# theori-io/nrsc5

Measured on AMD Instinct MI355X. Metric: IQ MS/s demod+decoded, higher is better.
Workload: dtype exact float32 half-band (== int16 Q15) / f32 OFDM + sync / int32 Viterbi metrics

## Files before the change

### nrsc5_amd/csrc/engine.hip

```cpp
#include <math.h>
#include <stdarg.h>
#include <stdio.h>
#include <stdlib.h>
#include <algorithm>
#include <atomic>
#include <new>
#include "engine_internal.h"

static_assert(sizeof(nrsc5hip_record) == sizeof(BlockRecord), "record ABI mismatch");
static_assert(sizeof(BlockRecord) % 8 == 0, "record alignment");

static thread_local char g_err[512] = "";
extern "C" const char *nrsc5hip_last_error(void) { return g_err; }
void nrsc5::set_last_error(const char *msg) { snprintf(g_err, sizeof(g_err), "%s", msg); }
int nrsc5::fail(int code, const char *fmt, ...)
{
    char m[sizeof(g_err)];
    va_list ap; va_start(ap, fmt); vsnprintf(m, sizeof(m), fmt, ap); va_end(ap);
    set_last_error(m);
    return code;
}
#ifndef NRSC5HIP_SOURCE_SHA
#define NRSC5HIP_SOURCE_SHA "unknown"
#endif
// ... 293 lines not shown
            if ((rc = dev_alloc(e, &db.l2_ring, S * (size_t)cfg->p1_slots))) break;
            if (hipMemset(db.l2_ring, 0, S * (size_t)cfg->p1_slots * sizeof(nrsc5hip_l2_frame)) != hipSuccess) { rc = NRSC5HIP_EHIP; break; }
            const size_t npx = S * (size_t)db.px_slots * 2, nam = cfg->am_enable ? S * (size_t)cfg->p1_slots * 9 : 0;
            if ((rc = dev_alloc(e, &db.l2_px_ring, npx))) break;
            if (hipMemset(db.l2_px_ring, 0, npx * sizeof(nrsc5hip_l2_frame)) != hipSuccess) { rc = NRSC5HIP_EHIP; break; }
            if (nam) {
                if ((rc = dev_alloc(e, &db.l2_am_ring, nam))) break;
                if (hipMemset(db.l2_am_ring, 0, nam * sizeof(nrsc5hip_l2_frame)) != hipSuccess) { rc = NRSC5HIP_EHIP; break; }
            }
        }
        db.am = nullptr; db.am_sym = nullptr; db.am_q = nullptr; db.am_vit = nullptr; db.am_dec = nullptr; db.am_k9meta = nullptr; db.am_job = nullptr; db.am_ckpt = nullptr; db.am_ber = nullptr; db.am_pids_stage = nullptr; db.am_pids_rec = nullptr; db.am_nvit = 1;
        if (cfg->am_enable) {
            if ((rc = dev_alloc(e, &db.am, S))) break;
            if ((rc = dev_alloc(e, &db.am_sym, S * 4 * AM_SYMS))) break;
            if ((rc = dev_alloc(e, &db.am_q, S * 3 * 2 * (size_t)AM_VIT))) break;
            db.am_nvit = cfg->p1_async ? NWIN : 1;
            const size_t ndec = cfg->p1_async ? NAUX : 1;
            if ((rc = dev_alloc(e, &db.am_vit, S * db.am_nvit * 2 * AM_VIT))) break;
            if ((rc = dev_alloc(e, &db.am_dec, ndec * S * (size_t)(8 * AM_DEC_P1 + AM_DEC_P3)))) break;
            if (cfg->p1_async && (rc = dev_alloc(e, &db.am_k9meta, ndec * S))) break;
            if ((rc = dev_alloc(e, &db.am_job, S * NWIN))) break;
            if ((rc = dev_alloc(e, &db.am_ber, S * (size_t)cfg->p1_slots))) break;
            if (cfg->p1_async && cfg->l2_feedback && (rc = dev_alloc(e, &db.am_ckpt, S * NWIN * 8))) break;
            if ((rc = dev_alloc(e, &db.am_pids_stage, S * NWIN * 8 * (size_t)(3 * PIDS_LEN)))) break;
            if ((rc = dev_alloc(e, &db.am_pids_rec, S * NWIN * 8))) break;
            if (hipMemset(db.am_pids_rec, 0xff, S * NWIN * 8 * sizeof(int)) != hipSuccess) { rc = NRSC5HIP_EHIP; break; }
            if (hipMemset(db.am_job, 0, S * NWIN * sizeof(AmJob)) != hipSuccess || hipMemset(db.am_ber, 0, S * (size_t)cfg->p1_slots * sizeof(float)) != hipSuccess) { rc = NRSC5HIP_EHIP; break; }
            std::vector<AmStream> ainit(S);
            for (size_t k = 0; k < S; k++) init_am_state(ainit[k]);
            if (hipMemcpy(db.am, ainit.data(), S * sizeof(AmStream), hipMemcpyHostToDevice) != hipSuccess ||
                hipMemset(db.am_q, 0, S * 3 * 2 * (size_t)AM_VIT) != hipSuccess || hipMemset(db.am_vit, 0, S * db.am_nvit * 2 * AM_VIT) != hipSuccess ||
                hipMemset(db.am_sym, 0, S * 4 * AM_SYMS) != hipSuccess) { rc = NRSC5HIP_EHIP; snprintf(g_err, sizeof(g_err), "AM state init failed"); break; }
        }
        db.sync_phase_cycles = nullptr;
        e->stage_bytes = 4u << 20; e->stage_ring_bytes = 1u << 20;
        if ((rc = dev_alloc(e, &e->stage_dev, e->stage_bytes))) break;
        if (!cfg->p1_async) {
            for (int k = 0; k < nrsc5hip_engine::NSTAGE && !rc; k++) {
                if ((rc = dev_alloc(e, &e->stage_dev2[k], e->stage_ring_bytes + 16))) break;
                void *sp = nullptr;
                if (hipHostMalloc((void **)&e->stage_pin[k], e->stage_ring_bytes + 16, hipHostMallocMapped) != hipSuccess ||
                    hipHostGetDevicePointer(&sp, e->stage_pin[k], 0) != hipSuccess ||
                    hipEventCreateWithFlags(&e->stage_ev[k], hipEventDisableTiming) != hipSuccess) { rc = NRSC5HIP_ENOMEM; snprintf(g_err, sizeof(g_err), "pinned staging allocation failed"); }
                e->stage_pin_dev[k] = (uint8_t *)sp;
                e->stage_busy[k] = false;
            }
            if (rc) break;
            if (S * (size_t)cfg->p1_slots <= 64) {
                const size_t nw = S * (size_t)cfg->p1_slots * P1_WORDS;
                void *mp = nullptr;
                if (hipHostMalloc((void **)&e->frames_host, nw * sizeof(uint32_t), hipHostMallocMapped) != hipSuccess ||
                    hipHostGetDevicePointer(&mp, e->frames_host, 0) != hipSuccess) { rc = NRSC5HIP_ENOMEM; snprintf(g_err, sizeof(g_err), "pinned frame mirror allocation failed"); break; }
                memset(e->frames_host, 0, nw * sizeof(uint32_t));
                db.p1_mirror = (uint32_t *)mp;
            }
            int prio_least = 0, prio_greatest = 0;
            (void)hipDeviceGetStreamPriorityRange(&prio_least, &prio_greatest);
            if (hipStreamCreateWithPriority(&e->ingest, hipStreamDefault, prio_greatest) != hipSuccess || hipEventCreateWithFlags(&e->ev_ingest, hipEventDisableTiming) != hipSuccess ||
                hipEventCreateWithFlags(&e->ev_main, hipEventDisableTiming) != hipSuccess ||
                hipEventCreateWithFlags(&e->ev_appended, hipEventDisableTiming) != hipSuccess) { rc = NRSC5HIP_EHIP; snprintf(g_err, sizeof(g_err), "ingest stream creation failed"); break; }
            e->ingest_dirty = false; e->main_stepped = false; e->main_appended = false; e->early_flush = 128u << 10;
            if ((rc = dev_alloc(e, &e->decim_ticket, 1))) break;
            if (hipMemset(e->decim_ticket, 0, sizeof(unsigned)) != hipSuccess) { rc = NRSC5HIP_EHIP; break; }
            for (int k = 0; k < 2 && !rc; k++) {
                void *dp = nullptr;
                if (hipHostMalloc((void **)&e->report_host[k], sizeof(StreamReport), hipHostMallocMapped) != hipSuccess ||
                    hipHostGetDevicePointer(&dp, e->report_host[k], 0) != hipSuccess) { rc = NRSC5HIP_ENOMEM; snprintf(g_err, sizeof(g_err), "pinned report allocation failed"); break; }
// ... 230 lines not shown
```

### nrsc5_amd/csrc/engine_stage.hip

```cpp
#include <algorithm>
#include <cmath>
#include "engine_internal.h"

extern "C" void nrsc5hip_debug_seam_totals(double out[8], int reset)
{
    for (int k = 0; k < 8; k++) { if (out) out[k] = g_seam[k]; if (reset) g_seam[k] = 0; }
}
extern "C" void nrsc5hip_debug_seam_counts(double out[6], int reset)
{
    for (int k = 0; k < 6; k++) { if (out) out[k] = g_seam[8 + k]; if (reset) g_seam[8 + k] = 0; }
}

extern "C" int nrsc5hip_stage_l2_index(nrsc5hip_engine *e, const uint8_t *bits, int nbits, int nframes, nrsc5hip_l2_frame *out, uint8_t *pdu_bytes, long long stride)
{
    ON_ENGINE_DEVICE(e);
    if (!e || !bits || !out || nbits < 1 || nframes < 1) FAIL(NRSC5HIP_EINVAL, "bad argument");
    const int words = (nbits + 31) / 32;
    std::vector<uint32_t> w((size_t)words * nframes, 0u);
    for (int f = 0; f < nframes; f++)
        for (int i = 0; i < nbits; i++) w[(size_t)f * words + (i >> 5)] |= (uint32_t)(bits[(size_t)f * nbits + i] & 1u) << (i & 31);
    DevTmp tw;
    HIPCHK(hipMalloc(&tw.p, w.size() * sizeof(uint32_t)));
    uint32_t *dw = (uint32_t *)tw.p;
    HIPCHK(hipMemcpy(dw, w.data(), w.size() * sizeof(uint32_t), hipMemcpyHostToDevice));
// ... 663 lines not shown
    case NRSC5HIP_TUNE_DEFER_WAIT:        e->defer_wait = value != 0; break;
    case NRSC5HIP_TUNE_DIRECT_DECIMATE:   e->direct_decimate = value != 0; break;
    case NRSC5HIP_TUNE_HOST_CAPTURE: {
        if (e->hc_stream >= 0) { int rc = hc_detach(e); if (rc) return rc; }
        if (!e->hc_pin) break;
        e->host_capture = value != 0;
        if (value >= 512) {
            uint8_t *np = nullptr; void *dp = nullptr;
            if (hipHostMalloc((void **)&np, (size_t)value << 10, hipHostMallocMapped) != hipSuccess || hipHostGetDevicePointer(&dp, np, 0) != hipSuccess) FAIL(NRSC5HIP_ENOMEM, "pinned capture allocation failed");
            (void)hipHostFree(e->hc_pin);
            e->hc_pin = np; e->hc_dev = (uint8_t *)dp; e->hc_cap = (size_t)value << 10;
        }
        break;
    }
    case NRSC5HIP_TUNE_MIXFFT_SYMS: {
        e->mixfft_syms = (value == 2 || value == 4 || value == 8 || value == 16 || value == 32 || (value >= 100 && value <= 140)) ? value : 1;
        if (e->mixfft_syms >= 100) {
            int lds_max = 65536;
#ifndef HIPEMU
            HIPCHK(hipDeviceGetAttribute(&lds_max, hipDeviceAttributeMaxSharedMemoryPerBlock, e->cfg.device));
#endif
            const int room_kib = (lds_max - 24 * 1024) / 1024;
            if (e->mixfft_syms - 100 > room_kib) e->mixfft_syms = 100 + std::max(room_kib, 0);
        }
        break;
    }
    case NRSC5HIP_TUNE_AM_SEGMENTS:       e->am_segments = std::min(std::max(value, 1), K9_GMAX); break;
    case NRSC5HIP_TUNE_AM_WARM:           e->am_warm = value > 0 ? K9_WARM : 0; e->am_runin = value > 0 ? K9_TB_RUNIN : 0; break;
    case NRSC5HIP_TUNE_SYNC_PHASES:
        if (value && !e->sync_phase_buf) {
            int rc = dev_alloc(e, &e->sync_phase_buf, 16); if (rc) return rc;
            HIPCHK(hipMemset(e->sync_phase_buf, 0, 16 * sizeof(long long)));
        }
        e->db.sync_phase_cycles = value ? e->sync_phase_buf : nullptr;
        break;
    default: FAIL(NRSC5HIP_EINVAL, "unknown knob %d", knob);
    }
    return 0;
}

extern "C" int nrsc5hip_debug_flow_stats(nrsc5hip_engine *e, long long stats[2])
{
    if (!e || !stats) return NRSC5HIP_EINVAL;
    stats[0] = e->flow_bursts; stats[1] = e->flow_steps;
    return 0;
}

extern "C" int nrsc5hip_debug_host_capture_stats(nrsc5hip_engine *e, long long stats[5])
{
    if (!e || !stats) return NRSC5HIP_EINVAL;
    stats[0] = e->hc_attaches; stats[1] = e->hc_detaches; stats[2] = e->hc_rebases; stats[3] = e->hc_stream; stats[4] = e->reports_folded;
    return 0;
}

extern "C" int nrsc5hip_debug_fwd_stats(nrsc5hip_engine *e, int stats[2])
{
    ON_ENGINE_DEVICE(e);
    if (!e || !stats) FAIL(NRSC5HIP_EINVAL, "null argument");
    HIPCHK(hipDeviceSynchronize());
    HIPCHK(hipMemcpy(stats, e->db.fwd_stats, 2 * sizeof(int), hipMemcpyDeviceToHost));
    return 0;
}

extern "C" int nrsc5hip_debug_tb_stats(nrsc5hip_engine *e, int stats[2])
{
    ON_ENGINE_DEVICE(e);
    if (!stats) FAIL(NRSC5HIP_EINVAL, "null argument");
// ... 24 lines not shown
```

### nrsc5_amd/csrc/kernels.h

```cpp
#pragma once
#include "nrsc5hip.h"
#include "nrsc5_dev.h"

namespace nrsc5 {

struct DevTables {
    const uint16_t *deint_lut;
    const uint16_t *pids_gather;
    const uint32_t *eq_cell;
    const uint16_t *eq_out;
    const uint32_t *scr_p1;
    const uint32_t *scr_pids;
    const float2 *twiddle;
    const float2 *twiddle_a;
    const float *shape;
    const int16_t *hb_q15;
    const int16_t *acq_q15;
    const uint32_t *px_delay_wide;
    const uint32_t *px_delay_narrow;
    const uint32_t *am_deint_p1;
    const uint32_t *am_deint_p3_ma3;
    const uint32_t *am_deint_p3_ma1;
    const int16_t *am_acq_q15;
    const float *am_shape;
// ... 1 lines not shown
};

struct DevBuffers {
    StreamState *state;
    StreamState *ckpt;
    c16 *q15;
    long long q15_cap;
    c16 *acq_win;
    c16 *acq_filt;
    int *acq_list;
    float2 *acq_sums;
    float2 *bins;
    float2 *cfo_snap;
    float *cfo_phase;
    int loop_exact;
    float2 *nco_tab;
    int nco_policy;
    int8_t *pm;
    int8_t *pids_stage;
    int *pids_rec;
    int *coded;
    uint32_t *dec;
    int nstreams_alloc;
    uint8_t *tbmap;
    int *fwd_meta;
    int *fwd_stats;
    int *tb_stats;
    uint32_t *p1_ring;
    uint32_t *p1_mirror;
    int p1_slots;
    BlockRecord *records;
    int rec_cap;
    int *counters;
    long long *sync_phase_cycles;
    int8_t *px_mem;
    int8_t *px_pair;
    int8_t *px_stage;
    PxJob *px_job;
    unsigned long long *px_dec;
    uint32_t *px_ring;
    int px_slots;
    AmStream *am;
    uint8_t *am_sym;
    uint8_t *am_q;
    int8_t *am_vit;
    int am_nvit;
    unsigned long long *am_dec;
    K9Meta *am_k9meta;
    unsigned *am_k9stats;
    AmJob *am_job;
    AmCkpt *am_ckpt;
    float *am_ber;
    int8_t *am_pids_stage;
    int *am_pids_rec;
    nrsc5hip_l2_frame *l2_ring;
    nrsc5hip_l2_frame *l2_px_ring;
    nrsc5hip_l2_frame *l2_am_ring;
};

struct StreamReport { int counters[4]; long long rd; int nblocks; int nrec; BlockRecord rec[4]; unsigned seq; unsigned pad; };
void launch_decimate_fm_cu8_stream(const DevTables &tb, const DevBuffers &db, int s, const uint8_t *iq, unsigned nbytes, unsigned *ticket, hipStream_t st);
void launch_stream_tail(const DevTables &tb, const DevBuffers &db, int s, int first_rec, StreamReport *out, unsigned seq, int do_pids, hipStream_t st);

void launch_decimate_fm_cu8(const DevTables &tb, const DevBuffers &db, int nstreams, const int *stream_ids,
                            const uint8_t *iq_base, long long iq_stride, const unsigned *nbytes, unsigned max_nbytes,
                            hipStream_t st);
// ... 107 lines not shown
```

### nrsc5_amd/csrc/sync_body.h

```cpp
#pragma once
#include <hip/hip_runtime.h>
#include "kernels.h"
#include "wave_ops.h"
#include "viterbi_wave.h"
#include "prepare_block.h"
#include "l2_header.h"
#include "fastmath.h"

namespace nrsc5 {

constexpr int NREF_MAX = 30;
constexpr int CFO_LO = -2 * PW, CFO_HI = 2 * PW;

__device__ inline int ref_bin(int r) { const int i = r >> 1; return (r & 1) ? UB1 - PW * i : LB0 + PW * i; }

constexpr uint32_t PAT_POS = (1u << 1) | (1u << 5) | (1u << 6) | (1u << 8) | (1u << 21);
constexpr uint32_t PAT_NEG = (1u << 0) | (1u << 2) | (1u << 3) | (1u << 4) | (1u << 9) | (1u << 13) | (1u << 14) | (1u << 20) | (1u << 22) | (1u << 31);
constexpr uint32_t NEEDLE_MASK = 0x7fu | (0xfu << 8) | (3u << 13) | (7u << 20) | (1u << 31);
constexpr uint32_t NEEDLE_VAL0 = (1u << 1) | (1u << 5) | (1u << 6) | (1u << 8) | (1u << 21);
__device__ inline uint32_t needle_val(unsigned rsid) { return NEEDLE_VAL0 | ((rsid >> 1) << 10) | ((((rsid >> 1) ^ rsid) & 1u) << 11); }

struct LoopGains { float alpha, beta; };
__device__ inline LoopGains loop_gains()
{
// ... 178 lines not shown

__device__ __forceinline__ float cell_error(float2 v)
{
    const float ix = v.x >= 0 ? 1.0f : -1.0f, iy = v.y >= 0 ? 1.0f : -1.0f;
    const float dx = ix - v.x, dy = iy - v.y;
    return dx * dx + dy * dy;
}

__device__ __forceinline__ void store_soft(int8_t *pm_blk, float2 v, int side, int part, int n, int k, float mult_lb, float mult_ub)
{
    const int part20 = side ? 19 - part : part;
    const float mult = side ? mult_ub : mult_lb;
    char2 o; o.x = (signed char)soft_bit(v.x, mult); o.y = (signed char)soft_bit(v.y, mult);
    *(char2 *)(pm_blk + n * 720 + part20 * 36 + (k - 1) * 2) = o;
}

__device__ __forceinline__ void store_px(int8_t *pair, float2 v, int side, int part, int n, int k, int ppb, int odd, float mult_lb, float mult_ub)
{
    const int nx1 = ppb == 11 ? 1 : 2;
    const int ch = (part - PM_PART) >= nx1 ? 1 : 0;
    const int count = ch ? 2 : nx1, q = part - PM_PART - (ch ? 2 : 0);
    const int per_sym = 72 * count, len = NSYM * per_sym;
    const int idx = side ? 36 * count + (count - 1 - q) * 36 + (k - 1) * 2 : q * 36 + (k - 1) * 2;
    const float mult = (side && !ch) ? mult_ub : mult_lb;
    char2 o; o.x = (signed char)soft_bit(v.x, mult); o.y = (signed char)soft_bit(v.y, mult);
    *(char2 *)(pair + (size_t)ch * 2 * PX_MAX + odd * len + n * per_sym + idx) = o;
}

#ifndef HIPEMU
#define SYNC_OCCUPANCY(NT) __attribute__((amdgpu_waves_per_eu((NT) > 512 ? 6 : 1, (NT) > 512 ? 6 : 8)))
#else
#define SYNC_OCCUPANCY(NT)
#endif
enum { PRE_STATE, PRE_BC, PRE_PXS, PRE_STARTED_PM, PRE_P1_COUNT, PRE_FINE_EPOCH, PRE_PM_SLOT, PRE_MER_CNT, PRE_ERR_LB, PRE_ERR_UB, PRE_N };
constexpr int SYNC_OFF_REFPH = NREF_MAX * NSYM * (int)sizeof(float2), SYNC_OFF_REFCS = SYNC_OFF_REFPH + NREF_MAX * NSYM * (int)sizeof(float);
constexpr int SYNC_OFF_CFO = SYNC_OFF_REFCS + NREF_MAX * NSYM * (int)sizeof(float2), SYNC_REF_BYTES = SYNC_OFF_CFO + (CFO_HI - CFO_LO) * 22;
template <int SYNC_NT> struct SyncLds {
    alignas(16) uint8_t lds_raw[SYNC_REF_BYTES > PM_BLOCK ? SYNC_REF_BYTES : PM_BLOCK];
    alignas(16) int8_t sh_pids_coded[3 * PIDS_LEN];
    double red[2][SYNC_NT / 64];
    long long sh_tstamp;
    float smag[NREF_MAX];
    int ref_ok[NREF_MAX], ref_bc[NREF_MAX], ref_psmi[NREF_MAX];
    int sh_i[8];
    float sh_f[8];
    float sh_diff[2 * 14];
    uint32_t sh_pids_out[4];
    int sh_seen[16 + 80];
    float ref_freq[NREF_MAX];
    int sh_pre[PRE_N];
    uint16_t sh_gather[PIDS_CODED];
};

template <int SYNC_NT>
__device__ __forceinline__ void sync_body(uint8_t *lds_base, const DevTables &tb, const DevBuffers &db, const int s, int parity, int slot, int fuse_prepare, int window, int pids_inline, int do_prepare, int ext_refs)
{
    SyncLds<SYNC_NT> &L = *reinterpret_cast<SyncLds<SYNC_NT> *>(lds_base);
    StreamState &st = db.state[s];
    if (do_prepare) {
        if (threadIdx.x == 0) prepare_block(db, st, s, false);
        __threadfence_block();
        __syncthreads();
    }
    const int tid = threadIdx.x;
    constexpr int NREFBIN = (NREF_MAX * NSYM + SYNC_NT - 1) / SYNC_NT;
    const int e_active = st.active, e_nblocks = st.nblocks, e_samperr = st.samperr_cur, e_psmi = st.psmi;
    int e_word = 0;
    {
        const int *w = &st.sync_state;
        w = tid == PRE_BC ? &st.bc : tid == PRE_PXS ? &st.px_started : tid == PRE_STARTED_PM ? &st.started_pm : tid == PRE_P1_COUNT ? &st.p1_count : w;
        w = tid == PRE_FINE_EPOCH ? &st.fine_epoch : tid == PRE_PM_SLOT ? &st.pm_slot : tid == PRE_MER_CNT ? &st.mer_cnt : w;
        w = tid == PRE_ERR_LB ? (const int *)&st.error_lb : tid == PRE_ERR_UB ? (const int *)&st.error_ub : w;
        if (tid < PRE_N) e_word = *w;
    }
    const int e_bc_v = st.bc;
    float2 e_bin[NREFBIN];
    constexpr int NCOMMON = 2 * (PM_PART + 1) * NSYM;
    {
        const float2 *bins0 = db.bins + (size_t)s * NSYM * LIVE_N;
#pragma unroll
        for (int i = 0; i < NREFBIN; i++) {
            int k = min(tid + i * SYNC_NT, NREF_MAX * NSYM - 1);
            if (!ext_refs) k = min(k, NCOMMON - 1);
            e_bin[i] = bins0[(k % NSYM) * LIVE_N + bin_to_live(ref_bin(k / NSYM))];
        }
    }
    const int e_l = bin_to_live(ref_bin(min(tid, NREF_MAX - 1)));
    const float e_freq = st.costas_freq[e_l], e_phase = st.costas_phase[e_l];
    if (!e_active) {
        if (fuse_prepare && threadIdx.x == 0) prepare_block(db, st, s, false);
        return;
    }
    const int e_gather = tb.pids_gather[(e_bc_v & 15) * PIDS_CODED + min(tid, PIDS_CODED - 1)];
    constexpr int SYNC_NW = SYNC_NT / 64;
    long long &sh_tstamp = L.sh_tstamp;
    if (db.sync_phase_cycles && s == 0 && tid == 0) sh_tstamp = (long long)clock64();
#define SYNC_MARK(i) do { if (db.sync_phase_cycles && s == 0 && tid == 0) { const long long now = (long long)clock64(); db.sync_phase_cycles[i] += now - sh_tstamp; sh_tstamp = now; } } while (0)

    constexpr int OFF_REFPH = SYNC_OFF_REFPH, OFF_REFCS = SYNC_OFF_REFCS, OFF_CFO = SYNC_OFF_CFO;
    uint8_t *lds_raw = L.lds_raw;
    float2 (*refz)[NSYM] = (float2 (*)[NSYM])lds_raw;
    float (*refph)[NSYM] = (float (*)[NSYM])(lds_raw + OFF_REFPH);
    float2 (*refcs)[NSYM] = (float2 (*)[NSYM])(lds_raw + OFF_REFCS);
    int8_t (*cfo_offs)[22] = (int8_t (*)[22])(lds_raw + OFF_CFO);
    int8_t *pm_tile = (int8_t *)lds_raw;
    static_assert(PM_BLOCK % 16 == 0 && PM_FRAME % 16 == 0, "soft-bit rows leave in 16-byte pieces");
    auto &smag = L.smag; auto &ref_ok = L.ref_ok; auto &ref_bc = L.ref_bc; auto &ref_psmi = L.ref_psmi; auto &sh_i = L.sh_i; auto &sh_f = L.sh_f; auto &red = L.red;
    auto &sh_diff = L.sh_diff; auto &sh_pids_coded = L.sh_pids_coded; auto &sh_pids_out = L.sh_pids_out; auto &sh_seen = L.sh_seen; auto &ref_freq = L.ref_freq;
    auto &sh_pre = L.sh_pre; auto &sh_gather = L.sh_gather;
    static_assert(SYNC_NW == SYNC_NT / 64, "one partial sum per wave");
    static_assert(PM_BLOCK <= 65536, "a gather index fits 16 bits");
    if (tid == 0) { sh_i[2] = 0; sh_i[3] = 0; }

    float2 *bins = db.bins + (size_t)s * NSYM * LIVE_N;
    const int nblocks0 = wave_uniform(e_nblocks);
    BlockRecord &rec = db.records[(size_t)s * db.rec_cap + (nblocks0 % db.rec_cap)];
    const LoopGains g = loop_gains();
    const int samperr = wave_uniform(e_samperr);
    const int ppb = partitions_for_psmi(wave_uniform(e_psmi));
    const int nref = 2 * (ppb + 1);

    {
        const int adj = SYM_N / 2 - samperr;
        if (adj != 0)
        for (int l = tid; l < LIVE_N; l += SYNC_NT) {
            const int b = live_to_bin(l);
            st.costas_phase[l] = (float)((double)st.costas_phase[l] - (adj * (b - FFT_N / 2)) * 2 * M_PI / FFT_N);
        }
    }
#pragma unroll
    for (int i = 0; i < NREFBIN; i++) {
        const int k = tid + i * SYNC_NT;
        if (k < nref * NSYM) {
            if (!ext_refs && k >= NCOMMON) e_bin[i] = bins[(k % NSYM) * LIVE_N + bin_to_live(ref_bin(k / NSYM))];
            refz[k / NSYM][k % NSYM] = e_bin[i];
        }
    }
    if (tid < PRE_N) sh_pre[tid] = e_word;
    if (tid < PIDS_CODED) sh_gather[tid] = (uint16_t)e_gather;
    __syncthreads();
    SYNC_MARK(0);

    const bool exact_blk = db.loop_exact == 2 || (db.loop_exact == 1 && sh_pre[PRE_STATE] != SYNC_FINE);
    if (tid < nref) {
        const int l = bin_to_live(ref_bin(tid));
        float f = e_freq, p = e_phase;
        if (SYM_N / 2 - samperr != 0) p = st.costas_phase[l];
        if (exact_blk) adjust_ref_exact<false>(refz[tid], 1, refph[tid], 1, f, p, 0, g);
        else costas_block<true>(refz[tid], 1, f, p, 0, g, refz[tid], refph[tid]);
        int l2 = l;
#ifndef HIPEMU
        asm volatile("" : "+v"(l2));
#endif
        st.costas_freq[l2] = f; st.costas_phase[l2] = p;
        ref_freq[tid] = f;
    }
    __syncthreads();
    SYNC_MARK(1);

    if (sh_pre[PRE_STATE] == SYNC_COARSE) {
        if (tid < nref) {
            uint32_t d = 0;
            for (int n = 0; n < NSYM; n++) if (refz[tid][n].x > 0) d |= 1u << n;
            const unsigned rsid = (30 - (tid >> 1)) & 3;
            const int ok = ((d & NEEDLE_MASK) == needle_val(rsid));
            const uint32_t dd = d ^ (d << 1);
            ref_ok[tid] = ok;
            ref_bc[tid] = (int)((((dd >> 16) & 1) << 3) | (((dd >> 17) & 1) << 2) | (((dd >> 18) & 1) << 1) | ((dd >> 19) & 1));
            ref_psmi[tid] = (int)((((dd >> 25) & 1) << 5) | (((dd >> 26) & 1) << 4) | (((dd >> 27) & 1) << 3) | (((dd >> 28) & 1) << 2) | (((dd >> 29) & 1) << 1) | ((dd >> 30) & 1));
        }
        __syncthreads();
        if (tid == 0) {
            int good = 0;
            int *seen_bc = sh_seen, *seen_psmi = sh_seen + 16;
            for (int k = 0; k < 16; k++) seen_bc[k] = 0;
            for (int k = 0; k < 64; k++) seen_psmi[k] = 0;
            for (int r = 0; r < nref; r++) if (ref_ok[r]) { good++; seen_bc[ref_bc[r]]++; seen_psmi[ref_psmi[r]]++; }
            int action = 0;
            if (good >= 4) {
                int maj_bc = -1, maj_psmi = -1;
                for (int v = 0; v < 16; v++) if (seen_bc[v] > good / 2) maj_bc = v;
                for (int v = 0; v < 16; v++) if (seen_psmi[v] > good / 2) maj_psmi = v;
                if (maj_bc >= 0 && maj_psmi >= 0) {
                    st.bc = maj_bc; st.psmi = maj_psmi;
                    rec.freq_offset = (float)(((double)st.prev_angle - 2 * M_PI * st.cfo) * 744187.5 / (2 * M_PI * FFT_N));
                    rec.flags |= REC_TO_FINE;
                    st.sync_state = SYNC_FINE; st.fine_epoch++;
                    st.started_pm = 0;
                    st.px_pos = 0; st.px_ready = 0; st.px_started = 0;
                    sh_i[4] = maj_bc; sh_i[5] = maj_psmi;
                    action = 1;
                }
            } else if (st.cfo_wait == 0) {
                action = 2;
            } else {
                st.cfo_wait--;
            }
            sh_i[0] = action;
        }
        __syncthreads();
        if (sh_i[0] == 2) {
            for (int k = tid; k < (CFO_HI - CFO_LO) * 22; k += SYNC_NT) (&cfo_offs[0][0])[k] = -1;
            __syncthreads();
            if constexpr (SYNC_NT >= LIVE_N) {
                const int l = tid < LIVE_N ? tid : LIVE_N - 1;
                const bool mine = tid < LIVE_N;
                const int b = live_to_bin(l);
                const bool lower = l < LIVE_HALF;
                float f = st.costas_freq[l], p = st.costas_phase[l];
                int rslot = -1;
                if (lower) { if ((b - LB0) % PW == 0 && (b - LB0) / PW <= ppb) rslot = 2 * ((b - LB0) / PW); }
                else { if ((UB1 - b) % PW == 0 && (UB1 - b) / PW <= ppb) rslot = 2 * ((UB1 - b) / PW) + 1; }
                const float2 *src = rslot >= 0 ? (const float2 *)&refz[rslot][0] : (const float2 *)(bins + l);
                const int stride = rslot >= 0 ? 1 : LIVE_N;
                float2 *snap = db.cfo_snap + ((size_t)s * LIVE_N + l) * (PM_PART + 1);
                if (mine && !exact_blk)
                for (int q = 0; q <= PM_PART; q++) {
                    const int i = lower ? (PM_PART - q) : q;
                    const int cfo = lower ? (b - LB0 - PW * i) : (b - UB1 + PW * i);
                    if (cfo < CFO_LO || cfo >= CFO_HI) continue;
                    const uint32_t d = costas_block<false>(src, stride, f, p, cfo, g, nullptr, nullptr);
                    cfo_offs[cfo - CFO_LO][2 * i + (lower ? 0 : 1)] = (int8_t)needle_search(d, (30 - i) & 3);
                    snap[q] = make_float2(f, p);
                }
                if (mine && exact_blk)
                for (int q = 0; q <= PM_PART; q++) {
                    const int i = lower ? (PM_PART - q) : q;
                    const int cfo = lower ? (b - LB0 - PW * i) : (b - UB1 + PW * i);
                    if (cfo < CFO_LO || cfo >= CFO_HI) continue;
                    const uint32_t d = adjust_ref_exact<true>(const_cast<float2 *>(src), stride, db.cfo_phase + (size_t)s * NSYM * LIVE_N + l, LIVE_N, f, p, cfo, g);
                    cfo_offs[cfo - CFO_LO][2 * i + (lower ? 0 : 1)] = (int8_t)needle_search(d, (30 - i) & 3);
                    snap[q] = make_float2(f, p);
                }
                __syncthreads();
                constexpr int NCAND = CFO_HI - CFO_LO;
                static_assert(NCAND <= 128, "two waves vote");
                int my_best = -1;
                if (tid < NCAND) {
                    int best = -1, best_count = 0;
                    for (int r = 0; r < 22; r++) {
                        const int v = cfo_offs[tid][r];
                        if (v < 0) continue;
                        int cnt = 0;
                        for (int r2 = 0; r2 < 22; r2++) cnt += cfo_offs[tid][r2] == v;
                        if (cnt > best_count || (cnt == best_count && v < best)) { best = v; best_count = cnt; }
                    }
                    if (best >= 0 && best_count >= 3) my_best = best;
                }
                if (tid < 128) {
                    const unsigned long long m = __ballot(my_best >= 0);
                    if ((tid & 63) == 0) { sh_seen[2 * (tid >> 6)] = (int)(uint32_t)m; sh_seen[2 * (tid >> 6) + 1] = (int)(uint32_t)(m >> 32); }
                    if (tid < NCAND) sh_seen[8 + tid] = my_best;
                }
                __syncthreads();
                if (tid == 0) {
                    int found = 0x7fffffff;
                    for (int w = 0; w < 4 && found == 0x7fffffff; w++) {
                        const uint32_t m = (uint32_t)sh_seen[w];
                        if (m) found = 32 * w + __ffs((int)m) - 1;
                    }
                    if (found != 0x7fffffff) {
                        const int best = sh_seen[8 + found];
                        st.keep_extra = ((NSYM - best) % NSYM) * SYM_N;
                        st.cfo += found + CFO_LO;
                        st.cfo_wait = 8;
                        found += CFO_LO;
                    }
                    sh_i[1] = found;
                }
                __syncthreads();
                {
                    const int last_cfo = sh_i[1];
                    int q_last = -1;
                    for (int q = 0; q <= PM_PART; q++) {
                        const int i = lower ? (PM_PART - q) : q;
                        const int cfo = lower ? (b - LB0 - PW * i) : (b - UB1 + PW * i);
                        if (cfo >= CFO_LO && cfo < CFO_HI && cfo <= last_cfo) q_last = q;
                    }
                    if (mine && q_last >= 0) { const float2 v = snap[q_last]; st.costas_freq[l] = v.x; st.costas_phase[l] = v.y; }
                }
            } else {
                for (int pass = 0; pass < 2; pass++) {
                    const int last_cfo = pass ? sh_i[1] : 0x7fffffff;
                    for (int l = tid; l < LIVE_N; l += SYNC_NT) {
                        const int b = live_to_bin(l);
                        const bool lower = l < LIVE_HALF;
                        float f = st.costas_freq[l], p = st.costas_phase[l];
                        int rslot = -1;
                        if (lower) { if ((b - LB0) % PW == 0 && (b - LB0) / PW <= ppb) rslot = 2 * ((b - LB0) / PW); }
                        else { if ((UB1 - b) % PW == 0 && (UB1 - b) / PW <= ppb) rslot = 2 * ((UB1 - b) / PW) + 1; }
                        const float2 *src = rslot >= 0 ? (const float2 *)&refz[rslot][0] : (const float2 *)(bins + l);
                        const int stride = rslot >= 0 ? 1 : LIVE_N;
                        bool visited = false;
                        for (int q = 0; q <= PM_PART; q++) {
                            const int i = lower ? (PM_PART - q) : q;
                            const int cfo = lower ? (b - LB0 - PW * i) : (b - UB1 + PW * i);
                            if (cfo < CFO_LO || cfo >= CFO_HI || cfo > last_cfo) continue;
                            const uint32_t d = costas_block<false>(src, stride, f, p, cfo, g, nullptr, nullptr);
                            visited = true;
                            if (pass == 0) cfo_offs[cfo - CFO_LO][2 * i + (lower ? 0 : 1)] = (int8_t)needle_search(d, (30 - i) & 3);
                        }
                        if (pass == 1 && visited) { st.costas_freq[l] = f; st.costas_phase[l] = p; }
                    }
                    if (pass == 1) break;
                    __syncthreads();
                    if (tid == 0) {
                        int found = 0x7fffffff;
                        for (int c = 0; c < CFO_HI - CFO_LO && found == 0x7fffffff; c++) {
                            int *count = sh_seen;
                            for (int k = 0; k < NSYM; k++) count[k] = 0;
                            for (int r = 0; r < 22; r++) if (cfo_offs[c][r] >= 0) count[cfo_offs[c][r]]++;
                            int best = -1, best_count = 0;
                            for (int k = 0; k < NSYM; k++) if (count[k] > best_count) { best = k; best_count = count[k]; }
                            if (best >= 0 && best_count >= 3) {
                                st.keep_extra = ((NSYM - best) % NSYM) * SYM_N;
                                st.cfo += c + CFO_LO;
                                st.cfo_wait = 8;
                                found = c + CFO_LO;
                            }
                        }
                        sh_i[1] = found;
                    }
                    __syncthreads();
                }
        }
            }
        __syncthreads();
    }

    SYNC_MARK(2);
    const bool locked_now = sh_pre[PRE_STATE] == SYNC_COARSE && sh_i[0] == 1;
    const int state_now = locked_now ? (int)SYNC_FINE : sh_pre[PRE_STATE];
    if (state_now == SYNC_FINE) {
        const int bc = locked_now ? sh_i[4] : sh_pre[PRE_BC];
        const int psmi_now = locked_now ? sh_i[5] : wave_uniform(e_psmi);
        const int pxs_now = locked_now ? 0 : sh_pre[PRE_PXS];
        const int ppb_px = routed_partitions_for_psmi(psmi_now);
        const bool px_on = ppb_px > PM_PART && (pxs_now || (bc & 1) == 0);
        for (int k = tid; k < nref * NSYM; k += SYNC_NT) {
            const int r = k / NSYM, n = k % NSYM;
            float sn, cs; fast_sincos(refph[r][n], sn, cs);
            refcs[r][n] = make_float2(cs, sn);
        }
        if (tid < nref) {
            float sum = 0.0f;
            for (int n = 0; n < NSYM; n++) sum += fabsf(refz[tid][n].x);
            smag[tid] = sum / NSYM;
        }
        if (tid >= 64 && tid < 64 + ppb) {
            const int i = tid - 64;
            sh_diff[2 * i] = half_turn_diff(refph[2 * i][0], refph[2 * (i + 1)][0]);
            sh_diff[2 * i + 1] = half_turn_diff(refph[2 * (i + 1) + 1][0], refph[2 * i + 1][0]);
        }
        __syncthreads();

        if (tid == 0) {
            float se = 0.0f, angle = 0.0f, sum_xy = 0.0f, sum_x2 = 0.0f;
            for (int i = 0; i < 2 * ppb; i++) se += sh_diff[i];
            se = (float)(se / (ppb * 2) * FFT_N / PW / (2 * M_PI));
            for (int i = 0; i <= ppb; i++) {
                float x = (float)(LB0 + PW * i - FFT_N / 2), y = ref_freq[2 * i];
                angle += y; sum_xy += x * y; sum_x2 += x * x;
                x = (float)(UB1 - PW * i - FFT_N / 2); y = ref_freq[2 * i + 1];
                angle += y; sum_xy += x * y; sum_x2 += x * x;
            }
            se = (float)(se - (sum_xy / sum_x2) * FFT_N / (2 * M_PI) * NSYM);
            st.samperr = (int)roundf(se);
            angle /= (ppb + 1) * 2;
            st.angle = angle;
            sh_f[0] = angle;
        }
        __syncthreads();
        if (tid < nref) st.costas_freq[bin_to_live(ref_bin(tid))] = ref_freq[tid] - sh_f[0];
        SYNC_MARK(3);

        const int ncell = 2 * ppb * NSYM * 18;
        constexpr int MP1C = 2 * PM_PART * NSYM * 18 / SYNC_NT;
        static_assert(MP1C * SYNC_NT == 2 * PM_PART * NSYM * 18, "the MP1 cells divide evenly over the work-items");
        float2 cellv[MP1C];
        double e_lb = 0.0, e_ub = 0.0;
        if (ppb == PM_PART) {
            uint32_t cw[MP1C];
#pragma unroll
            for (int i = 0; i < MP1C; i++) cw[i] = tb.eq_cell[tid + SYNC_NT * i];
#pragma unroll
            for (int i = 0; i < MP1C; i++) cellv[i] = bins[((cw[i] >> 10) & 31u) * LIVE_N + (cw[i] & 1023u)];
#pragma unroll
            for (int i = 0; i < MP1C; i++) {
                const uint32_t w = cw[i];
                const int n = (w >> 10) & 31u, r_lo = (w >> 15) & 31u, r_hi = (w >> 20) & 31u, k = (w >> 25) & 31u;
                const float2 z = cellv[i];
                const float2 lp = refcs[r_lo][n], up = refcs[r_hi][n];
                const float a = k * smag[r_hi], bq = (PW - k) * smag[r_lo];
                const float2 den = make_float2(a * up.x + bq * lp.x, a * up.y + bq * lp.y);
                const float2 C = cdiv(make_float2((float)PW, (float)PW), den);
                const float2 v = make_float2(z.x * C.x - z.y * C.y, z.x * C.y + z.y * C.x);
                cellv[i] = v;
                const float e = cell_error(v);
                if (w >> 30) e_ub += e; else e_lb += e;
            }
        } else {
            for (int c = tid; c < ncell; c += SYNC_NT) {
                int side;
                const float e = cell_error(equalise_cell<0>(c, ppb, bins, refcs, smag, side));
                if (side) e_ub += e; else e_lb += e;
            }
        }
        e_lb = wave_sum_f64_rf(e_lb); e_ub = wave_sum_f64_rf(e_ub);
        if ((tid & 63) == 0) { red[0][tid >> 6] = e_lb; red[1][tid >> 6] = e_ub; }
        __syncthreads();
        if (tid == 0) {
            double sl = 0.0, su = 0.0;
            for (int w = 0; w < SYNC_NW; w++) { sl += red[0][w]; su += red[1][w]; }
            const float error_lb = (float)sl, error_ub = (float)su;
            float acc_lb = __builtin_bit_cast(float, sh_pre[PRE_ERR_LB]) + error_lb, acc_ub = __builtin_bit_cast(float, sh_pre[PRE_ERR_UB]) + error_ub;
            int cnt = sh_pre[PRE_MER_CNT] + 1;
            if (cnt == 16) {
                const float signal = (float)(2 * NSYM * (ppb * 18) * cnt);
                rec.mer_lb = 10 * log10f(signal / acc_lb);
                rec.mer_ub = 10 * log10f(signal / acc_ub);
                rec.flags |= REC_MER;
                cnt = 0; acc_lb = 0; acc_ub = 0;
            }
            st.error_lb = acc_lb; st.error_ub = acc_ub; st.mer_cnt = cnt;
            const float mer_lb = 2.0f * NSYM * (float)(ppb * 18) / error_lb;
            const float mer_ub = 2.0f * NSYM * (float)(ppb * 18) / error_ub;
            sh_f[1] = fmaxf(fminf(mer_lb * 10, 127.0f), 1.0f);
            sh_f[2] = fmaxf(fminf(mer_ub * 10, 127.0f), 1.0f);
        }
        __syncthreads();
        const float mult_lb = sh_f[1], mult_ub = sh_f[2];
        SYNC_MARK(4);

        const int pm_slot = sh_pre[PRE_PM_SLOT];
        int8_t *pm_blk = db.pm + ((size_t)s * NPM + pm_slot) * PM_FRAME + (size_t)bc * PM_BLOCK;
        if (ppb == PM_PART) {
#pragma unroll
            for (int i = 0; i < MP1C; i++) {
                const int c = tid + SYNC_NT * i;
                const float mult = c >= ncell / 2 ? mult_ub : mult_lb;
                char2 o; o.x = (signed char)soft_bit(cellv[i].x, mult); o.y = (signed char)soft_bit(cellv[i].y, mult);
                *(char2 *)(pm_tile + tb.eq_out[c]) = o;
            }
            __syncthreads();
            for (int q = tid; q < PM_BLOCK / 16; q += SYNC_NT) ((uint4 *)pm_blk)[q] = ((const uint4 *)pm_tile)[q];
        } else {
            for (int c = tid; c < ncell; c += SYNC_NT) {
                int k, n, part, side;
                cell_coords<0>(c, ppb, side, part, n, k);
                if (part < PM_PART) store_soft(pm_blk, equalise_cell<0>(c, ppb, bins, refcs, smag, side), side, part, n, k, mult_lb, mult_ub);
                else if (px_on && part < ppb_px) store_px(db.px_pair + (size_t)s * 4 * PX_MAX, equalise_cell<0>(c, ppb, bins, refcs, smag, side), side, part, n, k, ppb_px, bc & 1, mult_lb, mult_ub);
            }
        }
        if (px_on && ppb_px > ppb) {
            const int p0 = ppb > PM_PART ? ppb : PM_PART, np = ppb_px - p0;
            for (int c = tid; c < 2 * np * NSYM * 18; c += SYNC_NT) {
                const int k = 1 + c % 18, n = (c / 18) % NSYM, part = p0 + (c / (18 * NSYM)) % np, side = c / (18 * NSYM * np);
                const int b = (side ? UB1 - PW * (part + 1) : LB0 + PW * part) + k;
                store_px(db.px_pair + (size_t)s * 4 * PX_MAX, bins[n * LIVE_N + bin_to_live(b)], side, part, n, k, ppb_px, bc & 1, mult_lb, mult_ub);
            }
        }
        __threadfence_block();
        __syncthreads();
        SYNC_MARK(5);

        int8_t *stage = db.pids_stage + (((size_t)s * NWIN + parity) * 16 + slot) * (3 * PIDS_LEN);
        const int8_t *pm_src = ppb == PM_PART ? pm_tile : pm_blk;
        if (pids_inline) {
            for (int n = tid; n < PIDS_CODED; n += SYNC_NT) sh_pids_coded[n + n / 5] = pm_src[!locked_now ? (int)sh_gather[n] : (int)tb.pids_gather[bc * PIDS_CODED + n]];
            for (int n = tid; n < PIDS_CODED / 5; n += SYNC_NT) sh_pids_coded[6 * n + 5] = 0;
            __syncthreads();
            if ((tid >> 6) == 1) {
                uint32_t *out = sh_pids_out;
                viterbi_k7_wave_compact<PIDS_LEN>(sh_pids_coded, nullptr, out);
                WAVE_LDS_FENCE();
// ... 18 lines not shown
            rec.flags |= REC_PIDS;
            rec.bc_decoded = bc;
            if (bc == 0) { started_pm = 1; st.started_pm = 1; }
            if (started_pm && bc == 15) {
                const int slot = e_p1_count % db.p1_slots;
                st.p1_count = e_p1_count + 1;
                st.p1_pending[parity] = 1; st.p1_slot[parity] = slot; st.p1_record[parity] = nblocks0 % db.rec_cap; st.p1_epoch[parity] = fine_epoch;
                st.p1_pmslot[parity] = pm_slot;
                st.p1_verdict[parity] = 0; st.p1_recabs[parity] = nblocks0; st.p1_window[parity] = window;
                sh_i[2] = 1;
                rec.p1_slot = slot; rec.flags |= REC_P1;
            }
            if (ppb_px > PM_PART) {
                if ((bc & 1) == 0) st.px_started = 1;
                if ((pxs_now || (bc & 1) == 0) && (bc & 1)) {
                    st.px_go = NSYM * 72 * (ppb_px == 11 ? 1 : 2);
                    st.px_nch = ppb_px == 14 ? 2 : 1;
                    st.px_record = nblocks0 % db.rec_cap;
                    if (st.px_ready || st.px_pos == 32 * st.px_go) {
                        st.px_slot = st.px_count % db.px_slots; st.px_count++;
                        rec.sis = (uint32_t)st.px_slot;
                        rec.flags |= REC_P3 | (ppb_px == 14 ? (uint32_t)REC_P4 : 0u);
                    } else st.px_slot = -1;
                }
            }
            st.bc = (bc + 1) % 16;
            st.last_pm_slot = pm_slot;
            if (bc == 15) st.pm_slot = (pm_slot + 1) % NPM;
        }
    }
    __syncthreads();
    SYNC_MARK(14);

    if (tid == 64) {
        if (st.nco_mode) {
            const float pr = st.nco_re, pi = st.nco_im;
            st.theta = atan2((double)pi, (double)pr);
            rec.phase_re = pr; rec.phase_im = pi;
        } else {
            double th = st.theta + (double)NSYM * SYM_N * st.dtheta;
            th -= 2 * M_PI * rint(th / (2 * M_PI));
            st.theta = th;
            rec.phase_re = (float)cos(th); rec.phase_im = (float)sin(th);
        }
    }
    if (tid == 0) {
        const int keep_extra = st.keep_extra, state = st.sync_state, cfo = st.cfo, bc_now = st.bc, psmi = st.psmi, cfo_wait = st.cfo_wait, next_samperr = st.samperr, nblocks = st.nblocks;
        const long long rd = st.rd;
        const float prev_angle = st.prev_angle, next_angle = st.angle;
        const int keep = SYM_N + (SYM_N / 2 - samperr) + keep_extra;
        st.keep_extra = 0;
        st.rd = rd + (WIN_N - keep);
        rec.state_after = state; rec.samperr = samperr; rec.cfo = cfo; rec.keep = keep;
        rec.bc = bc_now; rec.psmi = psmi; rec.cfo_wait = cfo_wait; rec.next_samperr = next_samperr;
        rec.prev_angle = prev_angle;
        rec.next_angle = next_angle;
        if (sh_i[3]) {
            rec.pids[0] = sh_pids_out[0]; rec.pids[1] = sh_pids_out[1]; rec.pids[2] = sh_pids_out[2];
            if (sh_pids_out[3]) rec.flags |= REC_PIDS_CRC;
        }
        st.nblocks = nblocks + 1;
        st.active = 0;
    }
    if (fuse_prepare && !db.ckpt) { __threadfence_block(); __syncthreads(); }
    if (db.ckpt) {
        __threadfence_block();
        __syncthreads();
        if (sh_i[2]) {
            const uint32_t *src = (const uint32_t *)&st;
            uint32_t *dst = (uint32_t *)(db.ckpt + (size_t)s * NWIN + parity);
            for (int k = tid; k < (int)(sizeof(StreamState) / 4); k += SYNC_NT) dst[k] = src[k];
        }
        __syncthreads();
    }
    if (tid == 0 && fuse_prepare) prepare_block(db, st, s, false);
    SYNC_MARK(7);
}

}
```

Measured before the change: 274,300.

## Cache sync-kernel stream state in LDS and shorten serial tail sections

Snapshots more per-stream sync state (cfo, keep_extra, samperr, angle, rd, etc.) into the shared preload array so the final single-thread record write reads LDS instead of global stream state. The costas phase rotation for non-reference bins moves off the critical path onto spare work-items alongside the reference adjustment, and the NCO/theta update is computed early in parallel. The diff sum uses wave readlane instead of an LDS array plus a barrier, the eq_cell loads are hoisted earlier, and pm_tile output offsets are computed arithmetically instead of via a lookup table. The profiling stream selection also becomes configurable. This adds register pressure and more complex state bookkeeping, with a risk of divergence from the previous state semantics.

After: 274,800, median of 3. About the same (+0.2%).

```diff
diff --git a/nrsc5_amd/csrc/engine.hip b/nrsc5_amd/csrc/engine.hip
--- a/nrsc5_amd/csrc/engine.hip
+++ b/nrsc5_amd/csrc/engine.hip
@@ -349,7 +349,7 @@
                 hipMemset(db.am_q, 0, S * 3 * 2 * (size_t)AM_VIT) != hipSuccess || hipMemset(db.am_vit, 0, S * db.am_nvit * 2 * AM_VIT) != hipSuccess ||
                 hipMemset(db.am_sym, 0, S * 4 * AM_SYMS) != hipSuccess) { rc = NRSC5HIP_EHIP; snprintf(g_err, sizeof(g_err), "AM state init failed"); break; }
         }
-        db.sync_phase_cycles = nullptr;
+        db.sync_phase_cycles = nullptr; db.sync_phase_stream = 0;
         e->stage_bytes = 4u << 20; e->stage_ring_bytes = 1u << 20;
         if ((rc = dev_alloc(e, &e->stage_dev, e->stage_bytes))) break;
         if (!cfg->p1_async) {
diff --git a/nrsc5_amd/csrc/engine_stage.hip b/nrsc5_amd/csrc/engine_stage.hip
--- a/nrsc5_amd/csrc/engine_stage.hip
+++ b/nrsc5_amd/csrc/engine_stage.hip
@@ -719,7 +719,8 @@
             int rc = dev_alloc(e, &e->sync_phase_buf, 16); if (rc) return rc;
             HIPCHK(hipMemset(e->sync_phase_buf, 0, 16 * sizeof(long long)));
         }
-        e->db.sync_phase_cycles = value ? e->sync_phase_buf : nullptr;
+        e->db.sync_phase_cycles = value > 0 ? e->sync_phase_buf : nullptr;
+        e->db.sync_phase_stream = value > 0 ? value - 1 : 0;
         break;
     default: FAIL(NRSC5HIP_EINVAL, "unknown knob %d", knob);
     }
diff --git a/nrsc5_amd/csrc/kernels.h b/nrsc5_amd/csrc/kernels.h
--- a/nrsc5_amd/csrc/kernels.h
+++ b/nrsc5_amd/csrc/kernels.h
@@ -57,6 +57,7 @@
     BlockRecord *records;
     int rec_cap;
     int *counters;
+    int sync_phase_stream;
     long long *sync_phase_cycles;
     int8_t *px_mem;
     int8_t *px_pair;
diff --git a/nrsc5_amd/csrc/sync_body.h b/nrsc5_amd/csrc/sync_body.h
--- a/nrsc5_amd/csrc/sync_body.h
+++ b/nrsc5_amd/csrc/sync_body.h
@@ -234,7 +234,8 @@
 #else
 #define SYNC_OCCUPANCY(NT)
 #endif
-enum { PRE_STATE, PRE_BC, PRE_PXS, PRE_STARTED_PM, PRE_P1_COUNT, PRE_FINE_EPOCH, PRE_PM_SLOT, PRE_MER_CNT, PRE_ERR_LB, PRE_ERR_UB, PRE_N };
+enum { PRE_STATE, PRE_BC, PRE_PXS, PRE_STARTED_PM, PRE_P1_COUNT, PRE_FINE_EPOCH, PRE_PM_SLOT, PRE_MER_CNT, PRE_ERR_LB, PRE_ERR_UB,
+       PRE_KEEP_EXTRA, PRE_CFO, PRE_CFO_WAIT, PRE_SAMPERR, PRE_ANGLE, PRE_PREV_ANGLE, PRE_RD_LO, PRE_RD_HI, PRE_N };
 constexpr int SYNC_OFF_REFPH = NREF_MAX * NSYM * (int)sizeof(float2), SYNC_OFF_REFCS = SYNC_OFF_REFPH + NREF_MAX * NSYM * (int)sizeof(float);
 constexpr int SYNC_OFF_CFO = SYNC_OFF_REFCS + NREF_MAX * NSYM * (int)sizeof(float2), SYNC_REF_BYTES = SYNC_OFF_CFO + (CFO_HI - CFO_LO) * 22;
 template <int SYNC_NT> struct SyncLds {
@@ -246,13 +247,15 @@
     int ref_ok[NREF_MAX], ref_bc[NREF_MAX], ref_psmi[NREF_MAX];
     int sh_i[8];
     float sh_f[8];
-    float sh_diff[2 * 14];
     uint32_t sh_pids_out[4];
     int sh_seen[16 + 80];
     float ref_freq[NREF_MAX];
     int sh_pre[PRE_N];
     uint16_t sh_gather[PIDS_CODED];
+    double sh_theta;
+    float sh_nco[2];
 };
+static_assert(sizeof(SyncLds<768>) <= 30720, "k_sync<768> no longer fits beside four traceback-walk workgroups");
 
 template <int SYNC_NT>
 __device__ __forceinline__ void sync_body(uint8_t *lds_base, const DevTables &tb, const DevBuffers &db, const int s, int parity, int slot, int fuse_prepare, int window, int pids_inline, int do_prepare, int ext_refs)
@@ -273,6 +276,8 @@
         w = tid == PRE_BC ? &st.bc : tid == PRE_PXS ? &st.px_started : tid == PRE_STARTED_PM ? &st.started_pm : tid == PRE_P1_COUNT ? &st.p1_count : w;
         w = tid == PRE_FINE_EPOCH ? &st.fine_epoch : tid == PRE_PM_SLOT ? &st.pm_slot : tid == PRE_MER_CNT ? &st.mer_cnt : w;
         w = tid == PRE_ERR_LB ? (const int *)&st.error_lb : tid == PRE_ERR_UB ? (const int *)&st.error_ub : w;
+        w = tid == PRE_KEEP_EXTRA ? &st.keep_extra : tid == PRE_CFO ? &st.cfo : tid == PRE_CFO_WAIT ? &st.cfo_wait : tid == PRE_SAMPERR ? &st.samperr : w;
+        w = tid == PRE_ANGLE ? (const int *)&st.angle : tid == PRE_PREV_ANGLE ? (const int *)&st.prev_angle : tid == PRE_RD_LO ? (const int *)&st.rd : tid == PRE_RD_HI ? (const int *)&st.rd + 1 : w;
         if (tid < PRE_N) e_word = *w;
     }
     const int e_bc_v = st.bc;
@@ -296,8 +301,8 @@
     const int e_gather = tb.pids_gather[(e_bc_v & 15) * PIDS_CODED + min(tid, PIDS_CODED - 1)];
     constexpr int SYNC_NW = SYNC_NT / 64;
     long long &sh_tstamp = L.sh_tstamp;
-    if (db.sync_phase_cycles && s == 0 && tid == 0) sh_tstamp = (long long)clock64();
-#define SYNC_MARK(i) do { if (db.sync_phase_cycles && s == 0 && tid == 0) { const long long now = (long long)clock64(); db.sync_phase_cycles[i] += now - sh_tstamp; sh_tstamp = now; } } while (0)
+    if (db.sync_phase_cycles && s == db.sync_phase_stream && tid == 0) sh_tstamp = (long long)clock64();
+#define SYNC_MARK(i) do { if (db.sync_phase_cycles && s == db.sync_phase_stream && tid == 0) { const long long now = (long long)clock64(); db.sync_phase_cycles[i] += now - sh_tstamp; sh_tstamp = now; } } while (0)
 
     constexpr int OFF_REFPH = SYNC_OFF_REFPH, OFF_REFCS = SYNC_OFF_REFCS, OFF_CFO = SYNC_OFF_CFO;
     uint8_t *lds_raw = L.lds_raw;
@@ -308,7 +313,7 @@
     int8_t *pm_tile = (int8_t *)lds_raw;
     static_assert(PM_BLOCK % 16 == 0 && PM_FRAME % 16 == 0, "soft-bit rows leave in 16-byte pieces");
     auto &smag = L.smag; auto &ref_ok = L.ref_ok; auto &ref_bc = L.ref_bc; auto &ref_psmi = L.ref_psmi; auto &sh_i = L.sh_i; auto &sh_f = L.sh_f; auto &red = L.red;
-    auto &sh_diff = L.sh_diff; auto &sh_pids_coded = L.sh_pids_coded; auto &sh_pids_out = L.sh_pids_out; auto &sh_seen = L.sh_seen; auto &ref_freq = L.ref_freq;
+    auto &sh_pids_coded = L.sh_pids_coded; auto &sh_pids_out = L.sh_pids_out; auto &sh_seen = L.sh_seen; auto &ref_freq = L.ref_freq;
     auto &sh_pre = L.sh_pre; auto &sh_gather = L.sh_gather;
     static_assert(SYNC_NW == SYNC_NT / 64, "one partial sum per wave");
     static_assert(PM_BLOCK <= 65536, "a gather index fits 16 bits");
@@ -322,14 +327,7 @@
     const int ppb = partitions_for_psmi(wave_uniform(e_psmi));
     const int nref = 2 * (ppb + 1);
 
-    {
-        const int adj = SYM_N / 2 - samperr;
-        if (adj != 0)
-        for (int l = tid; l < LIVE_N; l += SYNC_NT) {
-            const int b = live_to_bin(l);
-            st.costas_phase[l] = (float)((double)st.costas_phase[l] - (adj * (b - FFT_N / 2)) * 2 * M_PI / FFT_N);
-        }
-    }
+    const int adj = SYM_N / 2 - samperr;
 #pragma unroll
     for (int i = 0; i < NREFBIN; i++) {
         const int k = tid + i * SYNC_NT;
@@ -347,7 +345,7 @@
     if (tid < nref) {
         const int l = bin_to_live(ref_bin(tid));
         float f = e_freq, p = e_phase;
-        if (SYM_N / 2 - samperr != 0) p = st.costas_phase[l];
+        if (adj != 0) p = (float)((double)e_phase - (adj * (ref_bin(tid) - FFT_N / 2)) * 2 * M_PI / FFT_N);
         if (exact_blk) adjust_ref_exact<false>(refz[tid], 1, refph[tid], 1, f, p, 0, g);
         else costas_block<true>(refz[tid], 1, f, p, 0, g, refz[tid], refph[tid]);
         int l2 = l;
@@ -356,6 +354,27 @@
 #endif
         st.costas_freq[l2] = f; st.costas_phase[l2] = p;
         ref_freq[tid] = f;
+    }
+    if (tid >= 64) {
+        if (adj != 0)
+        for (int l = tid - 64; l < LIVE_N; l += SYNC_NT - 64) {
+            const int b = live_to_bin(l);
+            const int i = l < LIVE_HALF ? b - LB0 : UB1 - b;
+            if (i % PW == 0 && i / PW <= ppb) continue;
+            st.costas_phase[l] = (float)((double)st.costas_phase[l] - (adj * (b - FFT_N / 2)) * 2 * M_PI / FFT_N);
+        }
+        if (tid == 64) {
+            double th; float pr, pi;
+            if (st.nco_mode) {
+                pr = st.nco_re; pi = st.nco_im;
+                th = atan2((double)pi, (double)pr);
+            } else {
+                th = st.theta + (double)NSYM * SYM_N * st.dtheta;
+                th -= 2 * M_PI * rint(th / (2 * M_PI));
+                pr = (float)cos(th); pi = (float)sin(th);
+            }
+            L.sh_theta = th; L.sh_nco[0] = pr; L.sh_nco[1] = pi;
+        }
     }
     __syncthreads();
     SYNC_MARK(1);
@@ -396,7 +415,7 @@
             } else if (st.cfo_wait == 0) {
                 action = 2;
             } else {
-                st.cfo_wait--;
+                sh_pre[PRE_CFO_WAIT] = --st.cfo_wait;
             }
             sh_i[0] = action;
         }
@@ -463,9 +482,9 @@
                     }
                     if (found != 0x7fffffff) {
                         const int best = sh_seen[8 + found];
-                        st.keep_extra = ((NSYM - best) % NSYM) * SYM_N;
-                        st.cfo += found + CFO_LO;
-                        st.cfo_wait = 8;
+                        st.keep_extra = sh_pre[PRE_KEEP_EXTRA] = ((NSYM - best) % NSYM) * SYM_N;
+                        st.cfo = sh_pre[PRE_CFO] = st.cfo + found + CFO_LO;
+                        st.cfo_wait = sh_pre[PRE_CFO_WAIT] = 8;
                         found += CFO_LO;
                     }
                     sh_i[1] = found;
@@ -515,9 +534,9 @@
                             int best = -1, best_count = 0;
                             for (int k = 0; k < NSYM; k++) if (count[k] > best_count) { best = k; best_count = count[k]; }
                             if (best >= 0 && best_count >= 3) {
-                                st.keep_extra = ((NSYM - best) % NSYM) * SYM_N;
-                                st.cfo += c + CFO_LO;
-                                st.cfo_wait = 8;
+                                st.keep_extra = sh_pre[PRE_KEEP_EXTRA] = ((NSYM - best) % NSYM) * SYM_N;
+                                st.cfo = sh_pre[PRE_CFO] = st.cfo + c + CFO_LO;
+                                st.cfo_wait = sh_pre[PRE_CFO_WAIT] = 8;
                                 found = c + CFO_LO;
                             }
                         }
@@ -544,21 +563,33 @@
             float sn, cs; fast_sincos(refph[r][n], sn, cs);
             refcs[r][n] = make_float2(cs, sn);
         }
+        constexpr int MP1C = 2 * PM_PART * NSYM * 18 / SYNC_NT;
+        static_assert(MP1C * SYNC_NT == 2 * PM_PART * NSYM * 18, "the MP1 cells divide evenly over the work-items");
+        float2 cellv[MP1C];
+        uint32_t cw[MP1C];
+        if (ppb == PM_PART) {
+#pragma unroll
+            for (int i = 0; i < MP1C; i++) cw[i] = tb.eq_cell[tid + SYNC_NT * i];
+        }
         if (tid < nref) {
             float sum = 0.0f;
             for (int n = 0; n < NSYM; n++) sum += fabsf(refz[tid][n].x);
             smag[tid] = sum / NSYM;
         }
-        if (tid >= 64 && tid < 64 + ppb) {
-            const int i = tid - 64;
-            sh_diff[2 * i] = half_turn_diff(refph[2 * i][0], refph[2 * (i + 1)][0]);
-            sh_diff[2 * i + 1] = half_turn_diff(refph[2 * (i + 1) + 1][0], refph[2 * i + 1][0]);
-        }
-        __syncthreads();
-
-        if (tid == 0) {
-            float se = 0.0f, angle = 0.0f, sum_xy = 0.0f, sum_x2 = 0.0f;
-            for (int i = 0; i < 2 * ppb; i++) se += sh_diff[i];
+        if (tid >= SYNC_NT - 64) {
+            const int i = tid - (SYNC_NT - 64);
+            float d0 = 0.0f, d1 = 0.0f;
+            if (i < ppb) {
+                d0 = half_turn_diff(refph[2 * i][0], refph[2 * (i + 1)][0]);
+                d1 = half_turn_diff(refph[2 * (i + 1) + 1][0], refph[2 * i + 1][0]);
+            }
+            float se = 0.0f;
+            for (int j = 0; j < ppb; j++) {
+                se += __builtin_bit_cast(float, wave_readlane(__builtin_bit_cast(int, d0), j));
+                se += __builtin_bit_cast(float, wave_readlane(__builtin_bit_cast(int, d1), j));
+            }
+            if (i == 0) {
+            float angle = 0.0f, sum_xy = 0.0f, sum_x2 = 0.0f;
             se = (float)(se / (ppb * 2) * FFT_N / PW / (2 * M_PI));
             for (int i = 0; i <= ppb; i++) {
                 float x = (float)(LB0 + PW * i - FFT_N / 2), y = ref_freq[2 * i];
@@ -567,24 +598,20 @@
                 angle += y; sum_xy += x * y; sum_x2 += x * x;
             }
             se = (float)(se - (sum_xy / sum_x2) * FFT_N / (2 * M_PI) * NSYM);
-            st.samperr = (int)roundf(se);
+            const int next_samperr = (int)roundf(se);
             angle /= (ppb + 1) * 2;
-            st.angle = angle;
+            st.samperr = next_samperr; st.angle = angle;
+            sh_pre[PRE_SAMPERR] = next_samperr; sh_pre[PRE_ANGLE] = __builtin_bit_cast(int, angle);
             sh_f[0] = angle;
+        }
         }
         __syncthreads();
         if (tid < nref) st.costas_freq[bin_to_live(ref_bin(tid))] = ref_freq[tid] - sh_f[0];
         SYNC_MARK(3);
 
         const int ncell = 2 * ppb * NSYM * 18;
-        constexpr int MP1C = 2 * PM_PART * NSYM * 18 / SYNC_NT;
-        static_assert(MP1C * SYNC_NT == 2 * PM_PART * NSYM * 18, "the MP1 cells divide evenly over the work-items");
-        float2 cellv[MP1C];
         double e_lb = 0.0, e_ub = 0.0;
         if (ppb == PM_PART) {
-            uint32_t cw[MP1C];
-#pragma unroll
-            for (int i = 0; i < MP1C; i++) cw[i] = tb.eq_cell[tid + SYNC_NT * i];
 #pragma unroll
             for (int i = 0; i < MP1C; i++) cellv[i] = bins[((cw[i] >> 10) & 31u) * LIVE_N + (cw[i] & 1023u)];
 #pragma unroll
@@ -639,10 +666,11 @@
         if (ppb == PM_PART) {
 #pragma unroll
             for (int i = 0; i < MP1C; i++) {
-                const int c = tid + SYNC_NT * i;
-                const float mult = c >= ncell / 2 ? mult_ub : mult_lb;
+                int side, part, n, k;
+                cell_coords<PM_PART>(tid + SYNC_NT * i, PM_PART, side, part, n, k);
+                const float mult = side ? mult_ub : mult_lb;
                 char2 o; o.x = (signed char)soft_bit(cellv[i].x, mult); o.y = (signed char)soft_bit(cellv[i].y, mult);
-                *(char2 *)(pm_tile + tb.eq_out[c]) = o;
+                *(char2 *)(pm_tile + n * 720 + (side ? 19 - part : part) * 36 + (k - 1) * 2) = o;
             }
             __syncthreads();
             for (int q = tid; q < PM_BLOCK / 16; q += SYNC_NT) ((uint4 *)pm_blk)[q] = ((const uint4 *)pm_tile)[q];
@@ -727,22 +755,15 @@
     __syncthreads();
     SYNC_MARK(14);
 
-    if (tid == 64) {
-        if (st.nco_mode) {
-            const float pr = st.nco_re, pi = st.nco_im;
-            st.theta = atan2((double)pi, (double)pr);
-            rec.phase_re = pr; rec.phase_im = pi;
-        } else {
-            double th = st.theta + (double)NSYM * SYM_N * st.dtheta;
-            th -= 2 * M_PI * rint(th / (2 * M_PI));
-            st.theta = th;
-            rec.phase_re = (float)cos(th); rec.phase_im = (float)sin(th);
-        }
-    }
+    if (tid == 64) { st.theta = L.sh_theta; rec.phase_re = L.sh_nco[0]; rec.phase_im = L.sh_nco[1]; }
     if (tid == 0) {
-        const int keep_extra = st.keep_extra, state = st.sync_state, cfo = st.cfo, bc_now = st.bc, psmi = st.psmi, cfo_wait = st.cfo_wait, next_samperr = st.samperr, nblocks = st.nblocks;
-        const long long rd = st.rd;
-        const float prev_angle = st.prev_angle, next_angle = st.angle;
+        const bool locked = sh_pre[PRE_STATE] == SYNC_COARSE && sh_i[0] == 1;
+        const int state = locked ? (int)SYNC_FINE : sh_pre[PRE_STATE];
+        const int bc_in = locked ? sh_i[4] : sh_pre[PRE_BC], psmi = locked ? sh_i[5] : e_psmi;
+        const int bc_now = state == SYNC_FINE ? (bc_in + 1) % 16 : bc_in;
+        const int keep_extra = sh_pre[PRE_KEEP_EXTRA], cfo = sh_pre[PRE_CFO], cfo_wait = sh_pre[PRE_CFO_WAIT], next_samperr = sh_pre[PRE_SAMPERR], nblocks = nblocks0;
+        const long long rd = (long long)(((unsigned long long)(uint32_t)sh_pre[PRE_RD_HI] << 32) | (uint32_t)sh_pre[PRE_RD_LO]);
+        const float prev_angle = __builtin_bit_cast(float, sh_pre[PRE_PREV_ANGLE]), next_angle = __builtin_bit_cast(float, sh_pre[PRE_ANGLE]);
         const int keep = SYM_N + (SYM_N / 2 - samperr) + keep_extra;
         st.keep_extra = 0;
         st.rd = rd + (WIN_N - keep);
```
